# yeyupiaoling/VoiceprintRecognition-Pytorch

Measured on NVIDIA H100. Metric: embeddings/sec (3s@16kHz) ECAPA-TDNN, higher is better.
Workload: dtype f32

## Files before the change

voiceprintrecognition-pytorch_b200/csrc/api.cu:

```cuda
#include <cmath>
#include <cstdarg>
#include <cstdio>
#include <cstdlib>
#include <cstring>
#include <new>
#include <string>
#include <vector>

#include "kernels.cuh"


using namespace vpb;

struct vp_handle {
  int device = 0;
  std::string err;
  float* d_weights = nullptr;
  size_t weights_bytes = 0;
  char* d_arena = nullptr;
  size_t arena_bytes = 0;
  cudaStream_t cap_stream = nullptr;
  bool fe_set = false;
  vp_frontend_desc fe{};
  vp_frontend_options fe_opt{VP_FRAME_DEFAULT, 0, 1.0};
  float* d_window = nullptr;
  double2* d_twiddle = nullptr;
  int* d_mel_start = nullptr;
  int* d_mel_count = nullptr;
  int* d_mel_off = nullptr;
  float* d_mel_w = nullptr;
  float* d_dct = nullptr;
};

struct vp_program {
  vp_handle* h = nullptr;
  std::vector<vp_op> ops;
  std::vector<int> engines;
  size_t ws_bytes = 0, in_floats = 0, out_floats = 0;
  int launches = 0;
  int B = 0;
  cudaGraphExec_t gexec = nullptr;
  const float* g_feats = nullptr;
  float* g_emb = nullptr;
  char* g_arena = nullptr;
  int runs = 0, g_miss = 0;
  bool g_off = false;
  int n_slots = 0;
  size_t arena_need() const { return ws_bytes + (((size_t)n_slots * 4 + 255) & ~(size_t)255); }
  unsigned* slot(int32_t q) const { return q > 0 ? reinterpret_cast<unsigned*>(h->d_arena + ws_bytes) + (q - 1) : nullptr; }
};

static int fail(vp_handle* h, int code, const char* fmt, ...) {
  char buf[512];
// ... 80 lines not shown
  if (d->power != 1 && d->power != 2) return fail(h, VP_ERR_UNSUPPORTED, "power must be 1 or 2");
  if (d->use_log < 0 || d->use_log > 3) return fail(h, VP_ERR_INVALID, "use_log %d", d->use_log);
  if (d->post != 0 && d->post != 1) return fail(h, VP_ERR_INVALID, "post %d", d->post);
  if (d->post == 1) {
    if (d->kind != 1) return fail(h, VP_ERR_UNSUPPORTED, "MFCC needs stft framing");
    if (!dct) return fail(h, VP_ERR_INVALID, "MFCC needs the DCT matrix");
    if (d->n_mels > 128 || d->n_out < 1 || d->n_out > d->n_mels)
      return fail(h, VP_ERR_UNSUPPORTED, "MFCC: n_mels %d (<= 128), n_out %d (<= n_mels)", d->n_mels, d->n_out);
  }
  for (int m = 0; m < d->n_mels; ++m) {
    if (mel_count[m] < 0 || mel_start[m] < 0 || mel_start[m] + mel_count[m] > N / 2 + 1 || mel_off[m] < 0 ||
        mel_off[m] + mel_count[m] > n_w)
      return fail(h, VP_ERR_INVALID, "mel filter %d out of range", m);
  }
  CUDA_TRY(h, cudaSetDevice(h->device));
  free_frontend(h);
  std::vector<double2> tw(N);
  for (int k = 0; k < N; ++k) {
    double a = -2.0 * M_PI * (double)k / (double)N;
    tw[k] = make_double2(cos(a), sin(a));
  }
  const int F = d->n_mels;
  CUDA_TRY(h, cudaMalloc(&h->d_window, sizeof(float) * d->win_length));
  CUDA_TRY(h, cudaMalloc(&h->d_twiddle, sizeof(double2) * N));
  CUDA_TRY(h, cudaMalloc(&h->d_mel_start, sizeof(int) * F));
  CUDA_TRY(h, cudaMalloc(&h->d_mel_count, sizeof(int) * F));
  CUDA_TRY(h, cudaMalloc(&h->d_mel_off, sizeof(int) * F));
  CUDA_TRY(h, cudaMalloc(&h->d_mel_w, sizeof(float) * (n_w > 0 ? n_w : 1)));
  CUDA_TRY(h, cudaMemcpy(h->d_window, window, sizeof(float) * d->win_length, cudaMemcpyHostToDevice));
  CUDA_TRY(h, cudaMemcpy(h->d_twiddle, tw.data(), sizeof(double2) * N, cudaMemcpyHostToDevice));
  CUDA_TRY(h, cudaMemcpy(h->d_mel_start, mel_start, sizeof(int) * F, cudaMemcpyHostToDevice));
  CUDA_TRY(h, cudaMemcpy(h->d_mel_count, mel_count, sizeof(int) * F, cudaMemcpyHostToDevice));
  CUDA_TRY(h, cudaMemcpy(h->d_mel_off, mel_off, sizeof(int) * F, cudaMemcpyHostToDevice));
  if (n_w > 0) CUDA_TRY(h, cudaMemcpy(h->d_mel_w, mel_w, sizeof(float) * n_w, cudaMemcpyHostToDevice));
  if (d->post == 1) {
    CUDA_TRY(h, cudaMalloc(&h->d_dct, sizeof(float) * F * d->n_out));
    CUDA_TRY(h, cudaMemcpy(h->d_dct, dct, sizeof(float) * F * d->n_out, cudaMemcpyHostToDevice));
  }
  h->fe = *d;
  h->fe_opt = vp_frontend_options{VP_FRAME_DEFAULT, 0, 1.0};
  h->fe_set = true;
  return VP_OK;
}

int vp_frontend_set_options(vp_handle* h, const vp_frontend_options* o) {
  if (!h || !o) return fail(h, VP_ERR_INVALID, "null argument");
  if (!h->fe_set) return fail(h, VP_ERR_INVALID, "front-end not configured (vp_frontend_set)");
  const bool kaldi = h->fe.kind == 0;
  const int m = o->frame_mode;
  if (kaldi ? (m != VP_FRAME_DEFAULT && m != VP_FRAME_KALDI_REFLECT)
            : (m != VP_FRAME_DEFAULT && (m < VP_FRAME_STFT_CONSTANT || m > VP_FRAME_STFT_NOCENTER)))
    return fail(h, VP_ERR_INVALID, "frame mode %d does not fit front-end kind %d", m, h->fe.kind);
  if (o->pad < 0 || (kaldi && o->pad != 0)) return fail(h, VP_ERR_INVALID, "pad %d (kind 1 only, >= 0)", o->pad);
  if (!(o->spec_scale > 0.0) || !std::isfinite(o->spec_scale) || (kaldi && o->spec_scale != 1.0))
    return fail(h, VP_ERR_INVALID, "spec_scale %g (finite, > 0; 1 for kind 0)", o->spec_scale);
  h->fe_opt = *o;
  return VP_OK;
// ... 35 lines not shown
  size_t nblk = (T + FPB - 1) / FPB;
  size_t n = round4((size_t)B * nblk * vp_feature_dim(h));
  if (h->fe.post == 1) n += round4((size_t)B * nblk) + round4((size_t)B * T * h->fe.n_mels);
  return n;
}

static int run_frontend(vp_handle* h, int want_kind, int want_post, const float* wave, int B, int L, const int32_t* keep,
                        float* feats, float* scratch, cudaStream_t st, int stage = 0, float* ext_max = nullptr) {
  if (!h) return VP_ERR_INVALID;
  if (!h->fe_set) return fail(h, VP_ERR_INVALID, "front-end not configured (vp_frontend_set)");
  if (want_kind >= 0 && h->fe.kind != want_kind) return fail(h, VP_ERR_INVALID, "front-end kind mismatch");
  if (want_post >= 0 && h->fe.post != want_post) return fail(h, VP_ERR_INVALID, "front-end post-stage mismatch (vp_melspec vs vp_mfcc)");
  if ((stage != 2 && !wave) || (stage != 1 && !feats) || !scratch || B < 1) return fail(h, VP_ERR_INVALID, "null/empty argument");
  if (stage != 0 && (h->fe.post != 1 || !ext_max)) return fail(h, VP_ERR_INVALID, "two-stage calls are for the MFCC front-end");
  const char* len_err = frontend_length_error(h, L);
  if (*len_err) return fail(h, VP_ERR_INVALID, "waveform of %d samples: %s", L, len_err);
  const int T = vp_num_frames(h, L);
  if (T < 1) return fail(h, VP_ERR_INVALID, "waveform of %d samples is shorter than one frame (%d)", L, h->fe.win_length);
  CUDA_TRY(h, cudaSetDevice(h->device));
  FrontendParams p;
  p.wave = wave; p.feats = feats; p.partial = scratch;
  p.window = h->d_window; p.twiddle = h->d_twiddle;
  p.mel_start = h->d_mel_start; p.mel_count = h->d_mel_count; p.mel_off = h->d_mel_off; p.mel_w = h->d_mel_w;
  p.B = B; p.L = L; p.T = T; p.kind = h->fe.kind; p.N = h->fe.n_fft; p.WL = h->fe.win_length; p.hop = h->fe.hop;
  p.F = h->fe.n_mels; p.remove_dc = h->fe.remove_dc; p.power = h->fe.power; p.use_log = h->fe.use_log;
  p.fpb = FPB; p.nblk = (T + FPB - 1) / FPB;
  p.frame = h->fe_opt.frame_mode;
  p.pad = p.kind == 0 ? p.WL / 2 - p.hop / 2 : h->fe_opt.pad;
  p.spec_mult = h->fe.power == 2 ? h->fe_opt.spec_scale * h->fe_opt.spec_scale : h->fe_opt.spec_scale;
  p.preemph = h->fe.preemph; p.log_floor = h->fe.log_floor; p.db_mult = h->fe.db_mult; p.cta_max = nullptr;
  frontend_plan(p);
  if (h->fe.post == 1) {
    MfccParams m;
    float* cta_max = scratch + round4((size_t)B * p.nblk * h->fe.n_out);
    float* mel = cta_max + round4((size_t)B * p.nblk);
    p.feats = mel; p.partial = nullptr; p.cta_max = cta_max;
    m.mel = mel; m.cta_max = cta_max; m.dct = h->d_dct; m.feats = feats; m.partial = scratch;
    m.B = B; m.T = T; m.M = h->fe.n_mels; m.K = h->fe.n_out; m.fpb = FPB; m.nblk = p.nblk; m.n_max = B * p.nblk;
    m.top_db = h->fe.top_db;
    if (stage == 1) {
      CUDA_TRY(h, launch_frontend_mfcc_mel(p, ext_max, st));
    } else if (stage == 2) {
      m.cta_max = ext_max; m.n_max = 1;
      CUDA_TRY(h, launch_frontend_mfcc_finish(p, m, keep, st));
    } else {
      CUDA_TRY(h, launch_frontend_mfcc(p, m, keep, st));
    }
    return VP_OK;
  }
  CUDA_TRY(h, launch_frontend(p, keep, st));
  return VP_OK;
}

int vp_fbank(vp_handle* h, const float* wave, int32_t B, int32_t Lpad, const int32_t* keep, float* feats,
             float* scratch, void* stream) {
  return run_frontend(h, 0, 0, wave, B, Lpad, keep, feats, scratch, (cudaStream_t)stream);
}
int vp_melspec(vp_handle* h, const float* wave, int32_t B, int32_t Lpad, const int32_t* keep, float* feats,
               float* scratch, void* stream) {
  return run_frontend(h, 1, 0, wave, B, Lpad, keep, feats, scratch, (cudaStream_t)stream);
}
int vp_mfcc(vp_handle* h, const float* wave, int32_t B, int32_t Lpad, const int32_t* keep, float* feats,
            float* scratch, void* stream) {
  return run_frontend(h, 1, 1, wave, B, Lpad, keep, feats, scratch, (cudaStream_t)stream);
}

int vp_mfcc_mel(vp_handle* h, const float* wave, int32_t B, int32_t Lpad, float* scratch, float* max_out, void* stream) {
  return run_frontend(h, 1, 1, wave, B, Lpad, nullptr, nullptr, scratch, (cudaStream_t)stream, 1, max_out);
}
int vp_mfcc_finish(vp_handle* h, int32_t B, int32_t Lpad, const int32_t* keep, float* feats, float* scratch,
                   const float* max_in, void* stream) {
  return run_frontend(h, 1, 1, nullptr, B, Lpad, keep, feats, scratch, (cudaStream_t)stream, 2, const_cast<float*>(max_in));
// ... 579 lines not shown
```

voiceprintrecognition-pytorch_b200/csrc/frontend.cu:

```cuda
#include "kernels.cuh"

namespace vpb {

struct cd { double x, y; };
__device__ __forceinline__ cd cadd(cd a, cd b) { return {a.x + b.x, a.y + b.y}; }
__device__ __forceinline__ cd csub(cd a, cd b) { return {a.x - b.x, a.y - b.y}; }
__device__ __forceinline__ cd cmul(cd a, cd b) { return {a.x * b.x - a.y * b.y, a.x * b.y + a.y * b.x}; }
__device__ __forceinline__ cd cmi(cd a) { return {a.y, -a.x}; }
__device__ __forceinline__ cd ld2(const double2* p) { const double2 v = *p; return {v.x, v.y}; }
__device__ __forceinline__ void st2(double2* p, cd v) { *p = make_double2(v.x, v.y); }

__device__ __forceinline__ void group_sync(int g, int G) { asm volatile("bar.sync %0, %1;" ::"r"(g + 1), "r"(G) : "memory"); }

__global__ void __launch_bounds__(256) frontend_kernel(const __grid_constant__ FrontendParams p) {
  pdl_launch_dependents();
  pdl_wait();
  extern __shared__ __align__(16) unsigned char smem_raw[];
  const int N = p.N, WL = p.WL, F = p.F;
  const int G = p.G;
  const int NG = 256 / G;
  const int span = (p.fpb - 1) * p.hop + WL;

  double2* tw = reinterpret_cast<double2*>(smem_raw);
  double2* bufA = tw + N;
  double2* bufB = bufA + (size_t)NG * N;
  float* stage = reinterpret_cast<float*>(bufB + (size_t)NG * N);
  float* win = stage + ((span + 3) & ~3);
  float* means = win + ((WL + 3) & ~3);
  float* red = means + NG * 2;

  const int tid = threadIdx.x;
  const int b = blockIdx.y;
  const int f0 = blockIdx.x * p.fpb;
  const int g = tid / G;
  const int t = tid - g * G;
  float vmax = -INFINITY;
  const float* wv = p.wave + (size_t)b * p.L;

  const int q0 = f0 * p.hop;
  for (int i = tid; i < span; i += 256) {
    int s = q0 + i;
    if (p.kind == 1) {
      const int Lp = p.L + 2 * p.pad;
      if (p.frame != VP_FRAME_STFT_NOCENTER) s -= N / 2;
      if (p.frame == VP_FRAME_DEFAULT) {
        if (s < 0) s = -s;
        if (s >= Lp) s = 2 * (Lp - 1) - s;
      } else if (p.frame == VP_FRAME_STFT_REPLICATE) {
        s = min(max(s, 0), Lp - 1);
      } else if (p.frame == VP_FRAME_STFT_CIRCULAR) {
        if (s < 0) s += Lp;
        if (s >= Lp) s -= Lp;
      }
      s -= p.pad;
    } else if (p.frame == VP_FRAME_KALDI_REFLECT) {
      s -= p.pad;
      if (s < 0) s = -1 - s;
      if (s >= p.L) s = 2 * p.L - 1 - s;
    }
    stage[i] = (s >= 0 && s < p.L) ? __ldg(wv + s) : 0.f;
  }
  for (int i = tid; i < WL; i += 256) win[i] = __ldg(p.window + i);
  for (int i = tid; i < N; i += 256) tw[i] = __ldg(p.twiddle + i);
  __syncthreads();

  const int npairs = p.fpb / 2;
  double2* src0 = bufA + (size_t)g * N;
  double2* dst0 = bufB + (size_t)g * N;
  for (int pair = g; pair < npairs; pair += NG) {
    const int fa = f0 + pair * 2;
    const int oa = (fa - f0) * p.hop;
    const bool va = fa < p.T, vb = fa + 1 < p.T;
    if (!va) break;

    float ma = 0.f, mb = 0.f;
    if (p.kind == 0 && p.remove_dc) {
      const int w = t >> 5, lane = t & 31;
      if (G >= 64) {
        if (w < 2) {
          const int o = oa + w * p.hop;
          float s = 0.f;
          if (w == 0 || vb)
            for (int j = lane; j < WL; j += 32) s += stage[o + j];
          s = warp_sum(s);
          if (lane == 0) means[g * 2 + w] = s / (float)WL;
        }
      } else {
        for (int w2 = 0; w2 < 2; ++w2) {
          const int o = oa + w2 * p.hop;
          float s = 0.f;
          if (w2 == 0 || vb)
            for (int j = lane; j < WL; j += 32) s += stage[o + j];
          s = warp_sum(s);
          if (lane == 0) means[g * 2 + w2] = s / (float)WL;
        }
      }
      group_sync(g, G);
      ma = means[g * 2];
      mb = means[g * 2 + 1];
    }
    for (int j = t; j < N; j += G) {
      float ya = 0.f, yb = 0.f;
      if (j < WL) {
        const int jp = j > 0 ? j - 1 : 0;
        const float wj = win[j];
        {
          float x = stage[oa + j];
          if (p.kind == 0) {
            x = __fsub_rn(x, ma);
            if (p.preemph != 0.f) x = __fsub_rn(x, __fmul_rn(p.preemph, __fsub_rn(stage[oa + jp], ma)));
          }
          ya = __fmul_rn(x, wj);
        }
        if (vb) {
          float x = stage[oa + p.hop + j];
          if (p.kind == 0) {
            x = __fsub_rn(x, mb);
            if (p.preemph != 0.f) x = __fsub_rn(x, __fmul_rn(p.preemph, __fsub_rn(stage[oa + p.hop + jp], mb)));
          }
          yb = __fmul_rn(x, wj);
        }
      }
      src0[j] = make_double2((double)ya, (double)yb);
    }
    group_sync(g, G);

    double2* src = src0;
    double2* dst = dst0;
    int Ns = 1;
    for (int ps = 0; ps < p.n_pass; ++ps) {
      const int R = p.radix[ps];
      const int q = N / R;
      const int step = q / Ns;
      const bool pow2 = (Ns & (Ns - 1)) == 0;
      for (int j = t; j < q; j += G) {
        const int kk = pow2 ? (j & (Ns - 1)) : (j % Ns);
        const int base = (j - kk) * R + kk;
        if (R == 8) {
          cd v[8];
#pragma unroll
          for (int r = 0; r < 8; ++r) {
            v[r] = ld2(src + j + r * q);
            if (r > 0 && Ns > 1) v[r] = cmul(v[r], ld2(tw + r * kk * step));
          }
          const cd a0 = cadd(v[0], v[4]), a1 = csub(v[0], v[4]), a2 = cadd(v[2], v[6]), a3 = cmi(csub(v[2], v[6]));
          const cd a4 = cadd(v[1], v[5]), a5 = csub(v[1], v[5]), a6 = cadd(v[3], v[7]), a7 = cmi(csub(v[3], v[7]));
          const cd b0 = cadd(a0, a2), b2 = csub(a0, a2), b1 = cadd(a1, a3), b3 = csub(a1, a3);
          const cd b4 = cadd(a4, a6), b6 = cmi(csub(a4, a6));
          const double h = 0.70710678118654752440;
          const cd s5 = cadd(a5, a7), d5 = csub(a5, a7);
          const cd b5 = {h * (s5.x + s5.y), h * (s5.y - s5.x)};
          const cd b7 = {h * (d5.y - d5.x), -h * (d5.x + d5.y)};
          st2(dst + base, cadd(b0, b4));          st2(dst + base + Ns, cadd(b1, b5));
          st2(dst + base + 2 * Ns, cadd(b2, b6)); st2(dst + base + 3 * Ns, cadd(b3, b7));
          st2(dst + base + 4 * Ns, csub(b0, b4)); st2(dst + base + 5 * Ns, csub(b1, b5));
          st2(dst + base + 6 * Ns, csub(b2, b6)); st2(dst + base + 7 * Ns, csub(b3, b7));
        } else if (R == 4) {
          cd v0 = ld2(src + j), v1 = ld2(src + j + q), v2 = ld2(src + j + 2 * q), v3 = ld2(src + j + 3 * q);
          if (Ns > 1) {
            v1 = cmul(v1, ld2(tw + kk * step));
            v2 = cmul(v2, ld2(tw + 2 * kk * step));
            v3 = cmul(v3, ld2(tw + 3 * kk * step));
          }
          const cd a0 = cadd(v0, v2), a1 = csub(v0, v2), a2 = cadd(v1, v3), a3 = cmi(csub(v1, v3));
          st2(dst + base, cadd(a0, a2));          st2(dst + base + Ns, cadd(a1, a3));
          st2(dst + base + 2 * Ns, csub(a0, a2)); st2(dst + base + 3 * Ns, csub(a1, a3));
        } else if (R == 2) {
          const cd v0 = ld2(src + j);
          cd v1 = ld2(src + j + q);
          if (Ns > 1) v1 = cmul(v1, ld2(tw + kk * step));
          st2(dst + base, cadd(v0, v1));
          st2(dst + base + Ns, csub(v0, v1));
        } else {
          cd v[5];
#pragma unroll
          for (int r = 0; r < 5; ++r)
            if (r < R) {
              v[r] = ld2(src + j + r * q);
              if (r > 0 && Ns > 1) v[r] = cmul(v[r], ld2(tw + r * kk * step));
            }
#pragma unroll
          for (int m = 0; m < 5; ++m)
            if (m < R) {
              cd acc = v[0];
#pragma unroll
              for (int r = 1; r < 5; ++r)
                if (r < R) acc = cadd(acc, cmul(v[r], ld2(tw + ((r * m) % R) * q)));
              st2(dst + base + m * Ns, acc);
            }
        }
      }
      group_sync(g, G);
      double2* tmp = src; src = dst; dst = tmp;
      Ns *= R;
    }

    const int NB = N / 2 + 1;
    double* P = reinterpret_cast<double*>(dst);
    for (int k = t; k < NB; k += G) {
      const cd z = ld2(src + k);
      const cd zn = ld2(src + (k == 0 ? 0 : N - k));
      const double ar = 0.5 * (z.x + zn.x), ai = 0.5 * (z.y - zn.y);
      const double br = 0.5 * (z.y + zn.y), bi = -0.5 * (z.x - zn.x);
      double pa = ar * ar + ai * ai, pb = br * br + bi * bi;
      if (p.power == 1) { pa = sqrt(pa); pb = sqrt(pb); }
      if (p.spec_mult != 1.0) { pa *= p.spec_mult; pb *= p.spec_mult; }
      P[k] = pa;
      P[NB + k] = pb;
    }
    group_sync(g, G);

#pragma unroll
    for (int fr = 0; fr < 2; ++fr) {
      if (fr == 1 && !vb) break;
      const int f = fa + fr;
      const double* pf = P + fr * NB;
      for (int m = t; m < F; m += G) {
        const int st = __ldg(p.mel_start + m), cnt = __ldg(p.mel_count + m), off = __ldg(p.mel_off + m);
        double acc = 0.0;
        for (int i = 0; i < cnt; ++i) acc = fma(pf[st + i], (double)__ldg(p.mel_w + off + i), acc);
        float s = (float)acc;
        if (p.use_log == 1) s = logf(fmaxf(s, p.log_floor));
        else if (p.use_log == 2) s = p.db_mult * log10f(fmaxf(s, p.log_floor));
        else if (p.use_log == 3) s = logf(s + p.log_floor);
        vmax = fmaxf(vmax, s);
        p.feats[((size_t)b * p.T + f) * F + m] = s;
      }
    }
    group_sync(g, G);
  }
  __syncthreads();

  if (p.cta_max) {
    vmax = warp_max(vmax);
    if ((tid & 31) == 0) red[tid >> 5] = vmax;
    __syncthreads();
    if (tid == 0) {
      float m = red[0];
      for (int i = 1; i < 8; ++i) m = fmaxf(m, red[i]);
      p.cta_max[(size_t)b * p.nblk + blockIdx.x] = m;
    }
    return;
  }
  for (int m = tid; m < F; m += 256) {
    float s = 0.f;
    for (int f = f0; f < f0 + p.fpb && f < p.T; ++f) s += p.feats[((size_t)b * p.T + f) * F + m];
    p.partial[((size_t)b * p.nblk + blockIdx.x) * F + m] = s;
  }
}

__global__ void __launch_bounds__(256) mfcc_post_kernel(const __grid_constant__ MfccParams p) {
  pdl_launch_dependents();
  pdl_wait();
  extern __shared__ __align__(16) float sm[];
  float* dct = sm;
  float* tile = dct + p.M * p.K;
  float* outt = tile + p.fpb * p.M;
  float* red = outt + p.fpb * p.K;
  const int tid = threadIdx.x;
  const int b = blockIdx.y;
  const int f0 = blockIdx.x * p.fpb;
  float thr = -INFINITY;
  if (p.top_db >= 0.f) {
    float m = -INFINITY;
    for (int i = tid; i < p.n_max; i += 256) m = fmaxf(m, __ldg(p.cta_max + i));
    m = warp_max(m);
    if ((tid & 31) == 0) red[tid >> 5] = m;
    __syncthreads();
    m = red[0];
    for (int i = 1; i < 8; ++i) m = fmaxf(m, red[i]);
// ... 14 lines not shown
    for (int m = 0; m < p.M; ++m) s = fmaf(row[m], dct[m * p.K + k], s);
    outt[i] = s;
    if (f0 + fr < p.T) p.feats[((size_t)b * p.T + f0 + fr) * p.K + k] = s;
  }
  __syncthreads();
  for (int k = tid; k < p.K; k += 256) {
    float s = 0.f;
    for (int fr = 0; fr < p.fpb && f0 + fr < p.T; ++fr) s += outt[fr * p.K + k];
    p.partial[((size_t)b * p.nblk + blockIdx.x) * p.K + k] = s;
  }
}

__global__ void __launch_bounds__(128) cmn_mask_kernel(float* feats, const float* partial, const int* keep, int T, int F,
                                                       int nblk, int rows_per_cta) {
  pdl_launch_dependents();
  pdl_wait();
  const int b = blockIdx.y;
  const int kp = keep ? keep[b] : T;
  const int t0 = blockIdx.x * rows_per_cta;
  for (int m = threadIdx.x; m < F; m += blockDim.x) {
    float s = 0.f;
    for (int i = 0; i < nblk; ++i) s += partial[((size_t)b * nblk + i) * F + m];
    const float mean = s / (float)T;
    for (int t = t0; t < t0 + rows_per_cta && t < T; ++t) {
      float* q = feats + ((size_t)b * T + t) * F + m;
      *q = (t < kp) ? (*q - mean) : 0.f;
    }
  }
}

__global__ void __launch_bounds__(256) max_reduce_kernel(const float* v, int n, float* out) {
  pdl_launch_dependents();
  pdl_wait();
  __shared__ float red[8];
  float m = -INFINITY;
  for (int i = threadIdx.x; i < n; i += 256) m = fmaxf(m, v[i]);
  m = warp_max(m);
  if ((threadIdx.x & 31) == 0) red[threadIdx.x >> 5] = m;
  __syncthreads();
  if (threadIdx.x == 0) {
    m = red[0];
    for (int i = 1; i < 8; ++i) m = fmaxf(m, red[i]);
    out[0] = m;
  }
}

static int frontend_group_threads(int N) {
  const int first = (N % 8 == 0) ? 8 : 4;
  int G = ((N / first + 31) / 32) * 32;
  if (G < 32) G = 32;
  if (G > 256) G = 256;
  while (256 % G) G += 32;
  return G;
}

void frontend_plan(FrontendParams& p) {
  int n = p.N, k = 0;
  for (int r : {8, 4, 2, 5, 3})
    while (n % r == 0 && k < 12) { p.radix[k++] = r; n /= r; }
  p.n_pass = k;
  p.G = frontend_group_threads(p.N);
}

size_t frontend_smem_bytes(int N, int WL, int hop, int fpb) {
  const int G = frontend_group_threads(N);
  const int NG = 256 / G;
  const int span = (fpb - 1) * hop + WL;
  return sizeof(double2) * ((size_t)N + 2 * (size_t)NG * N) + sizeof(float) * (((span + 3) & ~3) + ((WL + 3) & ~3) + 2 * NG + 8 + 4);
}

static cudaError_t ensure_frontend_smem(size_t smem) {
  static PerDeviceSmem once;
  if (once.need(smem)) {
    cudaError_t e = cudaFuncSetAttribute(frontend_kernel, cudaFuncAttributeMaxDynamicSharedMemorySize, (int)smem);
    if (e != cudaSuccess) return e;
    once.set(smem);
  }
  return cudaSuccess;
}

cudaError_t launch_frontend_mfcc_mel(const FrontendParams& p, float* max_out, cudaStream_t stream) {
  size_t smem = frontend_smem_bytes(p.N, p.WL, p.hop, p.fpb);
  cudaError_t e = ensure_frontend_smem(smem);
  if (e != cudaSuccess) return e;
  dim3 grid(p.nblk, p.B);
  launch_pdl(frontend_kernel, grid, 256, smem, stream, p);
  e = cudaGetLastError();
  if (e != cudaSuccess) return e;
  launch_pdl(max_reduce_kernel, 1, 256, 0, stream, p.cta_max, p.B * p.nblk, max_out);
  return cudaGetLastError();
}

cudaError_t launch_frontend_mfcc_finish(const FrontendParams& p, const MfccParams& m, const int* keep, cudaStream_t stream) {
  dim3 grid(p.nblk, p.B);
  size_t smem2 = ((size_t)m.M * m.K + (size_t)m.fpb * (m.M + m.K) + 8) * sizeof(float);
  static PerDeviceSmem once;
  cudaError_t e;
  if (once.need(smem2)) {
    e = cudaFuncSetAttribute(mfcc_post_kernel, cudaFuncAttributeMaxDynamicSharedMemorySize, (int)smem2);
    if (e != cudaSuccess) return e;
    once.set(smem2);
  }
  launch_pdl(mfcc_post_kernel, grid, 256, smem2, stream, m);
  e = cudaGetLastError();
  if (e != cudaSuccess) return e;
  const int rows = 64;
  dim3 g2((p.T + rows - 1) / rows, p.B);
  launch_pdl(cmn_mask_kernel, g2, 128, 0, stream, m.feats, m.partial, keep, p.T, m.K, p.nblk, rows);
  return cudaGetLastError();
}

cudaError_t launch_frontend_mfcc(const FrontendParams& p, const MfccParams& m, const int* keep, cudaStream_t stream) {
  size_t smem = frontend_smem_bytes(p.N, p.WL, p.hop, p.fpb);
  cudaError_t e = ensure_frontend_smem(smem);
  if (e != cudaSuccess) return e;
  dim3 grid(p.nblk, p.B);
  launch_pdl(frontend_kernel, grid, 256, smem, stream, p);
  e = cudaGetLastError();
  if (e != cudaSuccess) return e;
  return launch_frontend_mfcc_finish(p, m, keep, stream);
}

cudaError_t launch_frontend(const FrontendParams& p, const int* keep, cudaStream_t stream) {
  size_t smem = frontend_smem_bytes(p.N, p.WL, p.hop, p.fpb);
  cudaError_t e = ensure_frontend_smem(smem);
  if (e != cudaSuccess) return e;
  dim3 grid(p.nblk, p.B);
  launch_pdl(frontend_kernel, grid, 256, smem, stream, p);
  e = cudaGetLastError();
  if (e != cudaSuccess) return e;
  const int rows = 64;
  dim3 g2((p.T + rows - 1) / rows, p.B);
  launch_pdl(cmn_mask_kernel, g2, 128, 0, stream, p.feats, p.partial, keep, p.T, p.F, p.nblk, rows);
  return cudaGetLastError();
}

}
```

voiceprintrecognition-pytorch_b200/csrc/kernels.cuh:

```cuda
#pragma once
#include "common.cuh"

namespace vpb {

struct FrontendParams {
  const float* wave; float* feats; float* partial;
  const float* window; const double2* twiddle;
  const int* mel_start; const int* mel_count; const int* mel_off; const float* mel_w;
  int B, L, T, kind, N, WL, hop, F, remove_dc, power, use_log, fpb, nblk;
  int frame;
  int pad;
  double spec_mult;
  float preemph, log_floor, db_mult;
  float* cta_max;
  int n_pass, radix[12], G;
};
void frontend_plan(FrontendParams& p);

struct MfccParams {
  const float* mel; const float* cta_max; const float* dct; float* feats; float* partial;
  int B, T, M, K, fpb, nblk, n_max;
  float top_db;
};

struct StatsParams {
  const float* src; float* dst;
  int B, R, C, in_ld, in_coff, out_ld, out_coff, mode, seg_len, n_seg;
  float eps;
};

struct AspParams {
  const float* x; const float* logit; float* dst;
  int B, T, C, x_ld, x_coff, l_ld, l_coff, out_ld, out_coff, mean_only;
  float eps;
};

struct EwParams {
  const float* x; const float* y; const float* att; const float* gate; const float* res; float* dst;
  long long rows; int C, rows_per_utt;
  int x_ld, x_coff, y_ld, y_coff, att_ld, att_coff, res_ld, res_coff, out_ld, out_coff, mode, act2;
// ... 14 lines not shown
int spectral_launches_tridiag(int n);
int apply_q_max_rows(int kz);
cudaError_t launch_spectral_laplacian(const float* emb, int n, int D, int n_drop, double* L, void* scratch, cudaStream_t stream);
cudaError_t launch_sym_tridiag(double* A, int n, double* d, double* e, double* tau, void* scratch, cudaStream_t stream);
cudaError_t launch_sym_tridiag_apply_q(const double* A, const double* tau, int n, double* Z, int kz, cudaStream_t stream);

size_t verify_scratch_bytes(int64_t n);
cudaError_t launch_verify_sort(const float* scores, const int32_t* labels, const int32_t* trial, const int32_t* enroll,
                               int64_t n_enroll, int64_t n, void* scratch, cudaStream_t stream);
cudaError_t launch_verify_curve(int64_t n, double p_target, double c_miss, double c_fa, void* scratch, float* sorted_scores,
                                uint8_t* sorted_labels, vp_verify_result* result, cudaStream_t stream);

cudaError_t launch_resample(const float* x, int64_t in_ld, float* y, int64_t out_ld, int B, const int64_t* n_in,
                            const int64_t* n_out, const int32_t* up, const int32_t* down, const int64_t* tap_off,
                            const double* taps, cudaStream_t stream);
size_t gain_scratch_bytes(int B, int64_t ld);
cudaError_t launch_gain(float* w, int64_t ld, int B, const int64_t* lens, double target_db, double max_gain_db,
                        int32_t* flags, void* scratch, cudaStream_t stream);

cudaError_t launch_frontend(const FrontendParams& p, const int* keep, cudaStream_t stream);
cudaError_t launch_frontend_mfcc(const FrontendParams& p, const MfccParams& m, const int* keep, cudaStream_t stream);
cudaError_t launch_frontend_mfcc_mel(const FrontendParams& p, float* max_out, cudaStream_t stream);
cudaError_t launch_frontend_mfcc_finish(const FrontendParams& p, const MfccParams& m, const int* keep, cudaStream_t stream);
size_t frontend_smem_bytes(int N, int WL, int hop, int fpb);
cudaError_t launch_conv_ffma(const ConvParams& p, cudaStream_t stream);
cudaError_t launch_conv_c1(const ConvParams& p, cudaStream_t stream);
cudaError_t launch_colstats(const StatsParams& p, cudaStream_t stream);
cudaError_t launch_asp_pool(const AspParams& p, cudaStream_t stream);
cudaError_t launch_ew(const EwParams& p, cudaStream_t stream);
bool conv_tc_supported(const ConvParams& p);
cudaError_t launch_conv_tc(const ConvParams& p, cudaStream_t stream);
bool conv_tc16_supported(const ConvParams& p);
cudaError_t launch_conv_tc16(const ConvParams& p, const float* w_tc16, float descale, cudaStream_t stream);

}
```

Measured before the change: 29300.

## Rewrite frontend FFT kernel with templated register FFT, padded smem and multi-tile CTAs

Reworks the fbank/mel frontend kernel: adds compile-time-N specializations that keep the FFT in registers with padded shared buffers and per-stage precomputed twiddles, caches mel weights and indices in shared memory, and loads constants via cp.async before the PDL wait. It also lets one CTA process several frame tiles, caching features in smem for the mean partials, and batches the mean-subtraction loop. The goal is to cut bank conflicts, global loads and launch/tail overhead in the feature extraction stage. It adds more shared memory per CTA, which may reduce occupancy.

```diff
diff --git a/voiceprintrecognition-pytorch_b200/csrc/api.cu b/voiceprintrecognition-pytorch_b200/csrc/api.cu
--- a/voiceprintrecognition-pytorch_b200/csrc/api.cu
+++ b/voiceprintrecognition-pytorch_b200/csrc/api.cu
@@ -28,7 +28,8 @@
   int* d_mel_start = nullptr;
   int* d_mel_count = nullptr;
   int* d_mel_off = nullptr;
-  float* d_mel_w = nullptr;
+  double* d_mel_w = nullptr;
+  int mel_nw = 0;
   float* d_dct = nullptr;
 };
 
@@ -155,17 +156,21 @@
   }
   const int F = d->n_mels;
   CUDA_TRY(h, cudaMalloc(&h->d_window, sizeof(float) * d->win_length));
-  CUDA_TRY(h, cudaMalloc(&h->d_twiddle, sizeof(double2) * N));
+  std::vector<double2> twx(N + 8);
+  frontend_twiddle_table(N, tw.data(), twx.data());
+  std::vector<double> mel_wd(mel_w, mel_w + (n_w > 0 ? n_w : 0));
+  CUDA_TRY(h, cudaMalloc(&h->d_twiddle, sizeof(double2) * (N + 8)));
   CUDA_TRY(h, cudaMalloc(&h->d_mel_start, sizeof(int) * F));
   CUDA_TRY(h, cudaMalloc(&h->d_mel_count, sizeof(int) * F));
   CUDA_TRY(h, cudaMalloc(&h->d_mel_off, sizeof(int) * F));
-  CUDA_TRY(h, cudaMalloc(&h->d_mel_w, sizeof(float) * (n_w > 0 ? n_w : 1)));
+  CUDA_TRY(h, cudaMalloc(&h->d_mel_w, sizeof(double) * (n_w > 0 ? n_w : 1)));
   CUDA_TRY(h, cudaMemcpy(h->d_window, window, sizeof(float) * d->win_length, cudaMemcpyHostToDevice));
-  CUDA_TRY(h, cudaMemcpy(h->d_twiddle, tw.data(), sizeof(double2) * N, cudaMemcpyHostToDevice));
+  CUDA_TRY(h, cudaMemcpy(h->d_twiddle, twx.data(), sizeof(double2) * (N + 8), cudaMemcpyHostToDevice));
   CUDA_TRY(h, cudaMemcpy(h->d_mel_start, mel_start, sizeof(int) * F, cudaMemcpyHostToDevice));
   CUDA_TRY(h, cudaMemcpy(h->d_mel_count, mel_count, sizeof(int) * F, cudaMemcpyHostToDevice));
   CUDA_TRY(h, cudaMemcpy(h->d_mel_off, mel_off, sizeof(int) * F, cudaMemcpyHostToDevice));
-  if (n_w > 0) CUDA_TRY(h, cudaMemcpy(h->d_mel_w, mel_w, sizeof(float) * n_w, cudaMemcpyHostToDevice));
+  if (n_w > 0) CUDA_TRY(h, cudaMemcpy(h->d_mel_w, mel_wd.data(), sizeof(double) * n_w, cudaMemcpyHostToDevice));
+  h->mel_nw = n_w > 0 ? n_w : 0;
   if (d->post == 1) {
     CUDA_TRY(h, cudaMalloc(&h->d_dct, sizeof(float) * F * d->n_out));
     CUDA_TRY(h, cudaMemcpy(h->d_dct, dct, sizeof(float) * F * d->n_out, cudaMemcpyHostToDevice));
@@ -247,6 +252,7 @@
   p.wave = wave; p.feats = feats; p.partial = scratch;
   p.window = h->d_window; p.twiddle = h->d_twiddle;
   p.mel_start = h->d_mel_start; p.mel_count = h->d_mel_count; p.mel_off = h->d_mel_off; p.mel_w = h->d_mel_w;
+  p.mel_nw = h->mel_nw;
   p.B = B; p.L = L; p.T = T; p.kind = h->fe.kind; p.N = h->fe.n_fft; p.WL = h->fe.win_length; p.hop = h->fe.hop;
   p.F = h->fe.n_mels; p.remove_dc = h->fe.remove_dc; p.power = h->fe.power; p.use_log = h->fe.use_log;
   p.fpb = FPB; p.nblk = (T + FPB - 1) / FPB;
@@ -254,12 +260,12 @@
   p.pad = p.kind == 0 ? p.WL / 2 - p.hop / 2 : h->fe_opt.pad;
   p.spec_mult = h->fe.power == 2 ? h->fe_opt.spec_scale * h->fe_opt.spec_scale : h->fe_opt.spec_scale;
   p.preemph = h->fe.preemph; p.log_floor = h->fe.log_floor; p.db_mult = h->fe.db_mult; p.cta_max = nullptr;
-  frontend_plan(p);
   if (h->fe.post == 1) {
     MfccParams m;
     float* cta_max = scratch + round4((size_t)B * p.nblk * h->fe.n_out);
     float* mel = cta_max + round4((size_t)B * p.nblk);
     p.feats = mel; p.partial = nullptr; p.cta_max = cta_max;
+    frontend_plan(p);
     m.mel = mel; m.cta_max = cta_max; m.dct = h->d_dct; m.feats = feats; m.partial = scratch;
     m.B = B; m.T = T; m.M = h->fe.n_mels; m.K = h->fe.n_out; m.fpb = FPB; m.nblk = p.nblk; m.n_max = B * p.nblk;
     m.top_db = h->fe.top_db;
@@ -273,6 +279,7 @@
     }
     return VP_OK;
   }
+  frontend_plan(p);
   CUDA_TRY(h, launch_frontend(p, keep, st));
   return VP_OK;
 }
diff --git a/voiceprintrecognition-pytorch_b200/csrc/frontend.cu b/voiceprintrecognition-pytorch_b200/csrc/frontend.cu
--- a/voiceprintrecognition-pytorch_b200/csrc/frontend.cu
+++ b/voiceprintrecognition-pytorch_b200/csrc/frontend.cu
@@ -10,35 +10,139 @@
 __device__ __forceinline__ cd ld2(const double2* p) { const double2 v = *p; return {v.x, v.y}; }
 __device__ __forceinline__ void st2(double2* p, cd v) { *p = make_double2(v.x, v.y); }
 
+__device__ __forceinline__ int xpad(int i) { return i + (i >> 3); }
+static int xpad_len(int N) { return N + (N >> 3); }
+
+template <int BYTES>
+__device__ __forceinline__ void cp_async(void* dst, const void* src) {
+  const unsigned d = (unsigned)__cvta_generic_to_shared(dst);
+  if (BYTES == 16) asm volatile("cp.async.cg.shared.global [%0], [%1], 16;" ::"r"(d), "l"(src) : "memory");
+  else asm volatile("cp.async.ca.shared.global [%0], [%1], %2;" ::"r"(d), "l"(src), "n"(BYTES) : "memory");
+}
+__device__ __forceinline__ void cp_async_wait_all() { asm volatile("cp.async.wait_all;" ::: "memory"); }
+
 __device__ __forceinline__ void group_sync(int g, int G) { asm volatile("bar.sync %0, %1;" ::"r"(g + 1), "r"(G) : "memory"); }
 
-__global__ void __launch_bounds__(256) frontend_kernel(const __grid_constant__ FrontendParams p) {
+__device__ __forceinline__ void bfly8(const cd* v, cd* o) {
+  const cd a0 = cadd(v[0], v[4]), a1 = csub(v[0], v[4]), a2 = cadd(v[2], v[6]), a3 = cmi(csub(v[2], v[6]));
+  const cd a4 = cadd(v[1], v[5]), a5 = csub(v[1], v[5]), a6 = cadd(v[3], v[7]), a7 = cmi(csub(v[3], v[7]));
+  const cd b0 = cadd(a0, a2), b2 = csub(a0, a2), b1 = cadd(a1, a3), b3 = csub(a1, a3);
+  const cd b4 = cadd(a4, a6), b6 = cmi(csub(a4, a6));
+  const double h = 0.70710678118654752440;
+  const cd s5 = cadd(a5, a7), d5 = csub(a5, a7);
+  const cd b5 = {h * (s5.x + s5.y), h * (s5.y - s5.x)};
+  const cd b7 = {h * (d5.y - d5.x), -h * (d5.x + d5.y)};
+  o[0] = cadd(b0, b4); o[1] = cadd(b1, b5); o[2] = cadd(b2, b6); o[3] = cadd(b3, b7);
+  o[4] = csub(b0, b4); o[5] = csub(b1, b5); o[6] = csub(b2, b6); o[7] = csub(b3, b7);
+}
+__device__ __forceinline__ void bfly4(const cd* v, cd* o) {
+  const cd a0 = cadd(v[0], v[2]), a1 = csub(v[0], v[2]), a2 = cadd(v[1], v[3]), a3 = cmi(csub(v[1], v[3]));
+  o[0] = cadd(a0, a2); o[1] = cadd(a1, a3); o[2] = csub(a0, a2); o[3] = csub(a1, a3);
+}
+__device__ __forceinline__ void bfly2(const cd* v, cd* o) {
+  o[0] = cadd(v[0], v[1]);
+  o[1] = csub(v[0], v[1]);
+}
+template <int R>
+__device__ __forceinline__ void bfly(const cd* v, cd* o) {
+  if (R == 8) bfly8(v, o);
+  else if (R == 4) bfly4(v, o);
+  else bfly2(v, o);
+}
+
+__host__ __device__ constexpr int pow2_radix(int rem) { return rem % 8 == 0 ? 8 : (rem % 4 == 0 ? 4 : 2); }
+__host__ __device__ constexpr int pow2_last_radix(int N) { return pow2_radix(N) == N ? N : pow2_last_radix(N / pow2_radix(N)); }
+__host__ __device__ constexpr int pow2_passes(int N) { return N == 1 ? 0 : 1 + pow2_passes(N / pow2_radix(N)); }
+
+template <int N, int Ns>
+__device__ __forceinline__ double2* fft_pow2(cd (&v)[8], double2* src, double2* dst, const double2* twx, int t, int g) {
+  constexpr int G = N / 8, R = pow2_radix(N / Ns), q = N / R, nb = 8 / R;
+  constexpr bool last = Ns * R == N;
+  if (Ns > 1) {
+#pragma unroll
+    for (int i = 0; i < nb; ++i)
+#pragma unroll
+      for (int r = 0; r < R; ++r) v[i * R + r] = ld2(src + xpad(t + i * G + r * q));
+  }
+#pragma unroll
+  for (int i = 0; i < nb; ++i) {
+    const int j = t + i * G;
+    const int kk = j & (Ns - 1);
+    if (Ns > 1) {
+#pragma unroll
+      for (int r = 1; r < R; ++r) v[i * R + r] = cmul(v[i * R + r], ld2(twx + (Ns - 1) + (r - 1) * Ns + kk));
+    }
+    cd o[R];
+    bfly<R>(&v[i * R], o);
+    const int base = (j - kk) * R + kk;
+#pragma unroll
+    for (int m = 0; m < R; ++m) {
+      v[i * R + m] = o[m];
+      if (!last) st2(dst + xpad(base + m * Ns), o[m]);
+      else if (i * G + m * Ns >= N / 2) st2(dst + j + m * Ns, o[m]);
+    }
+  }
+  group_sync(g, G);
+  if constexpr (last) return dst;
+  else return fft_pow2<N, Ns * R>(v, dst, src, twx, t, g);
+}
+
+__device__ __forceinline__ void split_power(const FrontendParams& p, cd z, cd zn, double& pa, double& pb) {
+  const double ar = 0.5 * (z.x + zn.x), ai = 0.5 * (z.y - zn.y);
+  const double br = 0.5 * (z.y + zn.y), bi = -0.5 * (z.x - zn.x);
+  pa = ar * ar + ai * ai;
+  pb = br * br + bi * bi;
+  if (p.power == 1) { pa = sqrt(pa); pb = sqrt(pb); }
+  if (p.spec_mult != 1.0) { pa *= p.spec_mult; pb *= p.spec_mult; }
+}
+
+template <int NFFT>
+__global__ void __launch_bounds__(256, 2) frontend_kernel(const __grid_constant__ FrontendParams p) {
   pdl_launch_dependents();
-  pdl_wait();
   extern __shared__ __align__(16) unsigned char smem_raw[];
-  const int N = p.N, WL = p.WL, F = p.F;
-  const int G = p.G;
+  const int N = NFFT ? NFFT : p.N, WL = p.WL, F = p.F;
+  const int G = NFFT ? NFFT / 8 : p.G;
   const int NG = 256 / G;
-  const int span = (p.fpb - 1) * p.hop + WL;
-
-  double2* tw = reinterpret_cast<double2*>(smem_raw);
-  double2* bufA = tw + N;
-  double2* bufB = bufA + (size_t)NG * N;
-  float* stage = reinterpret_cast<float*>(bufB + (size_t)NG * N);
+  const int cfr = p.fpb * p.tpc;
+  const int span = (cfr - 1) * p.hop + WL;
+  const int XN = N + (N >> 3);
+
+  double2* twx = reinterpret_cast<double2*>(smem_raw);
+  double2* roots = twx + N;
+  double2* bufs = roots + 8;
+  double* melw = reinterpret_cast<double*>(bufs + (size_t)NG * 2 * XN);
+  float* stage = reinterpret_cast<float*>(melw + ((p.mel_nw + 1) & ~1));
   float* win = stage + ((span + 3) & ~3);
-  float* means = win + ((WL + 3) & ~3);
+  float* fcache = win + ((WL + 3) & ~3);
+  int* melidx = reinterpret_cast<int*>(fcache + (p.cache ? (size_t)cfr * F : 0));
+  float* means = reinterpret_cast<float*>(melidx + 3 * F);
   float* red = means + NG * 2;
 
   const int tid = threadIdx.x;
   const int b = blockIdx.y;
-  const int f0 = blockIdx.x * p.fpb;
+  const int f0 = blockIdx.x * cfr;
   const int g = tid / G;
   const int t = tid - g * G;
   float vmax = -INFINITY;
   const float* wv = p.wave + (size_t)b * p.L;
 
+  for (int i = tid; i < N + 8; i += 256) cp_async<16>(twx + i, p.twiddle + i);
+  for (int i = tid; i < p.mel_nw; i += 256) cp_async<8>(melw + i, p.mel_w + i);
+  for (int i = tid; i < WL; i += 256) cp_async<4>(win + i, p.window + i);
+  for (int i = tid; i < F; i += 256) {
+    cp_async<4>(melidx + i, p.mel_start + i);
+    cp_async<4>(melidx + F + i, p.mel_count + i);
+    cp_async<4>(melidx + 2 * F + i, p.mel_off + i);
+  }
+  pdl_wait();
   const int q0 = f0 * p.hop;
-  for (int i = tid; i < span; i += 256) {
+  int i0 = 0;
+  if (p.kind == 0 && p.frame != VP_FRAME_KALDI_REFLECT && (reinterpret_cast<size_t>(wv + q0) & 15) == 0) {
+    const int n4 = min(span, p.L - q0) >> 2;
+    for (int i = tid; i < n4; i += 256) cp_async<16>(stage + 4 * i, wv + q0 + 4 * i);
+    i0 = n4 * 4;
+  }
+  for (int i = i0 + tid; i < span; i += 256) {
     int s = q0 + i;
     if (p.kind == 1) {
       const int Lp = p.L + 2 * p.pad;
@@ -60,13 +164,13 @@
     }
     stage[i] = (s >= 0 && s < p.L) ? __ldg(wv + s) : 0.f;
   }
-  for (int i = tid; i < WL; i += 256) win[i] = __ldg(p.window + i);
-  for (int i = tid; i < N; i += 256) tw[i] = __ldg(p.twiddle + i);
+  cp_async_wait_all();
   __syncthreads();
 
-  const int npairs = p.fpb / 2;
-  double2* src0 = bufA + (size_t)g * N;
-  double2* dst0 = bufB + (size_t)g * N;
+  const int npairs = cfr / 2;
+  double2* bufA = bufs + (size_t)g * 2 * XN;
+  double2* bufB = bufA + XN;
+  const int NB = N / 2 + 1;
   for (int pair = g; pair < npairs; pair += NG) {
     const int fa = f0 + pair * 2;
     const int oa = (fa - f0) * p.hop;
@@ -99,7 +203,7 @@
       ma = means[g * 2];
       mb = means[g * 2 + 1];
     }
-    for (int j = t; j < N; j += G) {
+    auto windowed = [&](int j) -> cd {
       float ya = 0.f, yb = 0.f;
       if (j < WL) {
         const int jp = j > 0 ? j - 1 : 0;
@@ -121,131 +225,168 @@
           yb = __fmul_rn(x, wj);
         }
       }
-      src0[j] = make_double2((double)ya, (double)yb);
+      return {(double)ya, (double)yb};
+    };
+
+    double* P;
+    if constexpr (NFFT != 0) {
+      cd v[8];
+#pragma unroll
+      for (int r = 0; r < 8; ++r) v[r] = windowed(t + r * (NFFT / 8));
+      const double2* zbuf = fft_pow2<NFFT, 1>(v, bufB, bufA, twx, t, g);
+      P = reinterpret_cast<double*>(zbuf == bufA ? bufB : bufA);
+      constexpr int LR = pow2_last_radix(NFFT), LNs = NFFT / LR;
+#pragma unroll
+      for (int i = 0; i < 8 / LR; ++i)
+#pragma unroll
+        for (int m = 0; m < LR; ++m) {
+          constexpr int Gc = NFFT / 8;
+          const int kb = i * Gc + m * LNs;
+          if (kb < NFFT / 2 || (kb == NFFT / 2 && t == 0)) {
+            const int k = t + kb;
+            const cd z = v[i * LR + m];
+            const cd zn = (k == 0 || kb == NFFT / 2) ? z : ld2(zbuf + (NFFT - k));
+            double pa, pb;
+            split_power(p, z, zn, pa, pb);
+            P[k] = pa;
+            P[NB + k] = pb;
+          }
+        }
+    } else {
+      for (int j = t; j < N; j += G) st2(bufA + xpad(j), windowed(j));
+      group_sync(g, G);
+      double2* src = bufA;
+      double2* dst = bufB;
+      int Ns = 1;
+      for (int ps = 0; ps < p.n_pass; ++ps) {
+        const int R = p.radix[ps];
+        const int q = N / R;
+        const bool pow2 = (Ns & (Ns - 1)) == 0;
+        for (int j = t; j < q; j += G) {
+          const int kk = pow2 ? (j & (Ns - 1)) : (j % Ns);
+          const int base = (j - kk) * R + kk;
+          const double2* tq = twx + (Ns - 1) + kk - Ns;
+          if (R == 8 || R == 4 || R == 2) {
+            cd v[8], o[8];
+#pragma unroll
+            for (int r = 0; r < 8; ++r)
+              if (r < R) {
+                v[r] = ld2(src + xpad(j + r * q));
+                if (r > 0 && Ns > 1) v[r] = cmul(v[r], ld2(tq + r * Ns));
+              }
+            if (R == 8) bfly8(v, o);
+            else if (R == 4) bfly4(v, o);
+            else bfly2(v, o);
+#pragma unroll
+            for (int m = 0; m < 8; ++m)
+              if (m < R) st2(dst + xpad(base + m * Ns), o[m]);
+          } else {
+            const double2* wr = roots + (R == 5 ? 0 : 5);
+            cd v[5];
+#pragma unroll
+            for (int r = 0; r < 5; ++r)
+              if (r < R) {
+                v[r] = ld2(src + xpad(j + r * q));
+                if (r > 0 && Ns > 1) v[r] = cmul(v[r], ld2(tq + r * Ns));
+              }
+#pragma unroll
+            for (int m = 0; m < 5; ++m)
+              if (m < R) {
+                cd acc = v[0];
+#pragma unroll
+                for (int r = 1; r < 5; ++r)
+                  if (r < R) acc = cadd(acc, cmul(v[r], ld2(wr + (r * m) % R)));
+                st2(dst + xpad(base + m * Ns), acc);
+              }
+          }
+        }
+        group_sync(g, G);
+        double2* tmp = src; src = dst; dst = tmp;
+        Ns *= R;
+      }
+      P = reinterpret_cast<double*>(dst);
+      for (int k = t; k < NB; k += G) {
+        double pa, pb;
+        split_power(p, ld2(src + xpad(k)), ld2(src + xpad(k == 0 ? 0 : N - k)), pa, pb);
+        P[k] = pa;
+        P[NB + k] = pb;
+      }
     }
     group_sync(g, G);
 
-    double2* src = src0;
-    double2* dst = dst0;
-    int Ns = 1;
-    for (int ps = 0; ps < p.n_pass; ++ps) {
-      const int R = p.radix[ps];
-      const int q = N / R;
-      const int step = q / Ns;
-      const bool pow2 = (Ns & (Ns - 1)) == 0;
-      for (int j = t; j < q; j += G) {
-        const int kk = pow2 ? (j & (Ns - 1)) : (j % Ns);
-        const int base = (j - kk) * R + kk;
-        if (R == 8) {
-          cd v[8];
-#pragma unroll
-          for (int r = 0; r < 8; ++r) {
-            v[r] = ld2(src + j + r * q);
-            if (r > 0 && Ns > 1) v[r] = cmul(v[r], ld2(tw + r * kk * step));
-          }
-          const cd a0 = cadd(v[0], v[4]), a1 = csub(v[0], v[4]), a2 = cadd(v[2], v[6]), a3 = cmi(csub(v[2], v[6]));
-          const cd a4 = cadd(v[1], v[5]), a5 = csub(v[1], v[5]), a6 = cadd(v[3], v[7]), a7 = cmi(csub(v[3], v[7]));
-          const cd b0 = cadd(a0, a2), b2 = csub(a0, a2), b1 = cadd(a1, a3), b3 = csub(a1, a3);
-          const cd b4 = cadd(a4, a6), b6 = cmi(csub(a4, a6));
-          const double h = 0.70710678118654752440;
-          const cd s5 = cadd(a5, a7), d5 = csub(a5, a7);
-          const cd b5 = {h * (s5.x + s5.y), h * (s5.y - s5.x)};
-          const cd b7 = {h * (d5.y - d5.x), -h * (d5.x + d5.y)};
-          st2(dst + base, cadd(b0, b4));          st2(dst + base + Ns, cadd(b1, b5));
-          st2(dst + base + 2 * Ns, cadd(b2, b6)); st2(dst + base + 3 * Ns, cadd(b3, b7));
-          st2(dst + base + 4 * Ns, csub(b0, b4)); st2(dst + base + 5 * Ns, csub(b1, b5));
-          st2(dst + base + 6 * Ns, csub(b2, b6)); st2(dst + base + 7 * Ns, csub(b3, b7));
-        } else if (R == 4) {
-          cd v0 = ld2(src + j), v1 = ld2(src + j + q), v2 = ld2(src + j + 2 * q), v3 = ld2(src + j + 3 * q);
-          if (Ns > 1) {
-            v1 = cmul(v1, ld2(tw + kk * step));
-            v2 = cmul(v2, ld2(tw + 2 * kk * step));
-            v3 = cmul(v3, ld2(tw + 3 * kk * step));
-          }
-          const cd a0 = cadd(v0, v2), a1 = csub(v0, v2), a2 = cadd(v1, v3), a3 = cmi(csub(v1, v3));
-          st2(dst + base, cadd(a0, a2));          st2(dst + base + Ns, cadd(a1, a3));
-          st2(dst + base + 2 * Ns, csub(a0, a2)); st2(dst + base + 3 * Ns, csub(a1, a3));
-        } else if (R == 2) {
-          const cd v0 = ld2(src + j);
-          cd v1 = ld2(src + j + q);
-          if (Ns > 1) v1 = cmul(v1, ld2(tw + kk * step));
-          st2(dst + base, cadd(v0, v1));
-          st2(dst + base + Ns, csub(v0, v1));
-        } else {
-          cd v[5];
-#pragma unroll
-          for (int r = 0; r < 5; ++r)
-            if (r < R) {
-              v[r] = ld2(src + j + r * q);
-              if (r > 0 && Ns > 1) v[r] = cmul(v[r], ld2(tw + r * kk * step));
-            }
-#pragma unroll
-          for (int m = 0; m < 5; ++m)
-            if (m < R) {
-              cd acc = v[0];
-#pragma unroll
-              for (int r = 1; r < 5; ++r)
-                if (r < R) acc = cadd(acc, cmul(v[r], ld2(tw + ((r * m) % R) * q)));
-              st2(dst + base + m * Ns, acc);
-            }
-        }
-      }
-      group_sync(g, G);
-      double2* tmp = src; src = dst; dst = tmp;
-      Ns *= R;
-    }
-
-    const int NB = N / 2 + 1;
-    double* P = reinterpret_cast<double*>(dst);
-    for (int k = t; k < NB; k += G) {
-      const cd z = ld2(src + k);
-      const cd zn = ld2(src + (k == 0 ? 0 : N - k));
-      const double ar = 0.5 * (z.x + zn.x), ai = 0.5 * (z.y - zn.y);
-      const double br = 0.5 * (z.y + zn.y), bi = -0.5 * (z.x - zn.x);
-      double pa = ar * ar + ai * ai, pb = br * br + bi * bi;
-      if (p.power == 1) { pa = sqrt(pa); pb = sqrt(pb); }
-      if (p.spec_mult != 1.0) { pa *= p.spec_mult; pb *= p.spec_mult; }
-      P[k] = pa;
-      P[NB + k] = pb;
-    }
-    group_sync(g, G);
-
-#pragma unroll
-    for (int fr = 0; fr < 2; ++fr) {
-      if (fr == 1 && !vb) break;
-      const int f = fa + fr;
-      const double* pf = P + fr * NB;
-      for (int m = t; m < F; m += G) {
-        const int st = __ldg(p.mel_start + m), cnt = __ldg(p.mel_count + m), off = __ldg(p.mel_off + m);
+    auto emit = [&](int o, double acc) {
+      const int fr = o >= F, m = o - fr * F;
+      float s = (float)acc;
+      if (p.use_log == 1) s = logf(fmaxf(s, p.log_floor));
+      else if (p.use_log == 2) s = p.db_mult * log10f(fmaxf(s, p.log_floor));
+      else if (p.use_log == 3) s = logf(s + p.log_floor);
+      vmax = fmaxf(vmax, s);
+      p.feats[((size_t)b * p.T + fa + fr) * F + m] = s;
+      if (p.cache) fcache[(size_t)(fa + fr - f0) * F + m] = s;
+    };
+    constexpr int MU = 4;
+    if (NFFT == 0 || 2 * F <= G) {
+      for (int o = t; o < 2 * F && (o < F || vb); o += G) {
+        const int fr = o >= F, m = o - fr * F;
+        const double* pf = P + fr * NB + melidx[m];
+        const double* wf = melw + melidx[2 * F + m];
+        const int cnt = melidx[F + m];
         double acc = 0.0;
-        for (int i = 0; i < cnt; ++i) acc = fma(pf[st + i], (double)__ldg(p.mel_w + off + i), acc);
-        float s = (float)acc;
-        if (p.use_log == 1) s = logf(fmaxf(s, p.log_floor));
-        else if (p.use_log == 2) s = p.db_mult * log10f(fmaxf(s, p.log_floor));
-        else if (p.use_log == 3) s = logf(s + p.log_floor);
-        vmax = fmaxf(vmax, s);
-        p.feats[((size_t)b * p.T + f) * F + m] = s;
-      }
-    }
-    group_sync(g, G);
+        for (int i = 0; i < cnt; ++i) acc = fma(pf[i], wf[i], acc);
+        emit(o, acc);
+      }
+    } else {
+      for (int o0 = t; o0 < 2 * F; o0 += MU * G) {
+        const double* pf[MU];
+        const double* wf[MU];
+        int cnt[MU], cmax = 0;
+        double acc[MU];
+#pragma unroll
+        for (int u = 0; u < MU; ++u) {
+          const int o = o0 + u * G, fr = o >= F;
+          const bool live = o < 2 * F && (!fr || vb);
+          const int m = live ? o - fr * F : 0;
+          pf[u] = P + fr * NB + melidx[m];
+          wf[u] = melw + melidx[2 * F + m];
+          cnt[u] = live ? melidx[F + m] : 0;
+          cmax = max(cmax, cnt[u]);
+          acc[u] = 0.0;
+        }
+        for (int i = 0; i < cmax; ++i)
+#pragma unroll
+          for (int u = 0; u < MU; ++u)
+            if (i < cnt[u]) acc[u] = fma(pf[u][i], wf[u][i], acc[u]);
+#pragma unroll
+        for (int u = 0; u < MU; ++u) {
+          const int o = o0 + u * G;
+          if (o < 2 * F && (o < F || vb)) emit(o, acc[u]);
+        }
+      }
+    }
+    if (NFFT == 0 || pow2_passes(NFFT ? NFFT : 1) % 2 == 0) group_sync(g, G);
   }
   __syncthreads();
 
+  const int blk0 = blockIdx.x * p.tpc;
   if (p.cta_max) {
     vmax = warp_max(vmax);
     if ((tid & 31) == 0) red[tid >> 5] = vmax;
     __syncthreads();
-    if (tid == 0) {
+    if (tid < p.tpc && blk0 + tid < p.nblk) {
       float m = red[0];
       for (int i = 1; i < 8; ++i) m = fmaxf(m, red[i]);
-      p.cta_max[(size_t)b * p.nblk + blockIdx.x] = m;
+      p.cta_max[(size_t)b * p.nblk + blk0 + tid] = m;
     }
     return;
   }
-  for (int m = tid; m < F; m += 256) {
+  for (int i = tid; i < p.tpc * F; i += 256) {
+    const int ti = i / F, m = i - ti * F;
+    if (blk0 + ti >= p.nblk) break;
+    const int fb = f0 + ti * p.fpb;
     float s = 0.f;
-    for (int f = f0; f < f0 + p.fpb && f < p.T; ++f) s += p.feats[((size_t)b * p.T + f) * F + m];
-    p.partial[((size_t)b * p.nblk + blockIdx.x) * F + m] = s;
+    for (int f = fb; f < fb + p.fpb && f < p.T; ++f)
+      s += p.cache ? fcache[(size_t)(f - f0) * F + m] : p.feats[((size_t)b * p.T + f) * F + m];
+    p.partial[((size_t)b * p.nblk + blk0 + ti) * F + m] = s;
   }
 }
 
@@ -306,9 +447,15 @@
     float s = 0.f;
     for (int i = 0; i < nblk; ++i) s += partial[((size_t)b * nblk + i) * F + m];
     const float mean = s / (float)T;
-    for (int t = t0; t < t0 + rows_per_cta && t < T; ++t) {
-      float* q = feats + ((size_t)b * T + t) * F + m;
-      *q = (t < kp) ? (*q - mean) : 0.f;
+    const int t1 = min(t0 + rows_per_cta, T);
+    for (int tb = t0; tb < t1; tb += 16) {
+      float v[16];
+#pragma unroll
+      for (int u = 0; u < 16; ++u)
+        if (tb + u < t1 && tb + u < kp) v[u] = feats[((size_t)b * T + tb + u) * F + m];
+#pragma unroll
+      for (int u = 0; u < 16; ++u)
+        if (tb + u < t1) feats[((size_t)b * T + tb + u) * F + m] = (tb + u < kp) ? (v[u] - mean) : 0.f;
     }
   }
 }
@@ -338,38 +485,72 @@
   return G;
 }
 
+static int plan_radices(int N, int* radix) {
+  int n = N, k = 0;
+  for (int r : {8, 4, 2, 5, 3})
+    while (n % r == 0 && k < 12) { radix[k++] = r; n /= r; }
+  return k;
+}
+
+void frontend_twiddle_table(int N, const double2* tw, double2* out) {
+  int radix[12];
+  const int n_pass = plan_radices(N, radix);
+  int Ns = 1;
+  for (int ps = 0; ps < n_pass; Ns *= radix[ps++])
+    for (int r = 1; r < radix[ps]; ++r)
+      for (int kk = 0; kk < Ns; ++kk) out[(Ns - 1) + (r - 1) * Ns + kk] = tw[r * kk * (N / (Ns * radix[ps]))];
+  out[N - 1] = make_double2(0.0, 0.0);
+  for (int k = 0; k < 8; ++k) {
+    const int R = k < 5 ? 5 : 3, e = k < 5 ? k : k - 5;
+    out[N + k] = (N % R == 0) ? tw[e * (N / R)] : make_double2(0.0, 0.0);
+  }
+}
+
+static size_t frontend_smem_bytes(const FrontendParams& p, int tpc, bool cache) {
+  const int NG = 256 / p.G;
+  const int cfr = p.fpb * tpc;
+  const int span = (cfr - 1) * p.hop + p.WL;
+  return sizeof(double2) * ((size_t)p.N + 8 + 2 * (size_t)NG * xpad_len(p.N)) + sizeof(double) * ((p.mel_nw + 1) & ~1) +
+         sizeof(float) * (((span + 3) & ~3) + ((p.WL + 3) & ~3) + (cache ? (size_t)cfr * p.F : 0) + 3 * p.F + 2 * NG + 8);
+}
+
 void frontend_plan(FrontendParams& p) {
-  int n = p.N, k = 0;
-  for (int r : {8, 4, 2, 5, 3})
-    while (n % r == 0 && k < 12) { p.radix[k++] = r; n /= r; }
-  p.n_pass = k;
+  p.n_pass = plan_radices(p.N, p.radix);
   p.G = frontend_group_threads(p.N);
-}
-
-size_t frontend_smem_bytes(int N, int WL, int hop, int fpb) {
-  const int G = frontend_group_threads(N);
-  const int NG = 256 / G;
-  const int span = (fpb - 1) * hop + WL;
-  return sizeof(double2) * ((size_t)N + 2 * (size_t)NG * N) + sizeof(float) * (((span + 3) & ~3) + ((WL + 3) & ~3) + 2 * NG + 8 + 4);
-}
-
-static cudaError_t ensure_frontend_smem(size_t smem) {
+  const size_t half_sm = (228 * 1024 - 2 * 1024) / 2, cta_max = 227 * 1024;
+  const bool want = p.cta_max == nullptr;
+  p.tpc = 1;
+  p.cache = want && frontend_smem_bytes(p, 1, true) <= cta_max;
+  for (int tpc : {4, 2})
+    if (tpc <= p.nblk && frontend_smem_bytes(p, tpc, want) <= half_sm) { p.tpc = tpc; p.cache = want; break; }
+}
+
+template <int NFFT>
+static cudaError_t launch_frontend_kernel_n(const FrontendParams& p, size_t smem, cudaStream_t stream) {
   static PerDeviceSmem once;
   if (once.need(smem)) {
-    cudaError_t e = cudaFuncSetAttribute(frontend_kernel, cudaFuncAttributeMaxDynamicSharedMemorySize, (int)smem);
+    cudaError_t e = cudaFuncSetAttribute(frontend_kernel<NFFT>, cudaFuncAttributeMaxDynamicSharedMemorySize, (int)smem);
     if (e != cudaSuccess) return e;
     once.set(smem);
   }
-  return cudaSuccess;
+  dim3 grid((p.nblk + p.tpc - 1) / p.tpc, p.B);
+  launch_pdl(frontend_kernel<NFFT>, grid, 256, smem, stream, p);
+  return cudaGetLastError();
+}
+
+static cudaError_t launch_frontend_kernel(const FrontendParams& p, cudaStream_t stream) {
+  const size_t smem = frontend_smem_bytes(p, p.tpc, p.cache);
+  switch (p.N) {
+    case 256: return launch_frontend_kernel_n<256>(p, smem, stream);
+    case 512: return launch_frontend_kernel_n<512>(p, smem, stream);
+    case 1024: return launch_frontend_kernel_n<1024>(p, smem, stream);
+    case 2048: return launch_frontend_kernel_n<2048>(p, smem, stream);
+    default: return launch_frontend_kernel_n<0>(p, smem, stream);
+  }
 }
 
 cudaError_t launch_frontend_mfcc_mel(const FrontendParams& p, float* max_out, cudaStream_t stream) {
-  size_t smem = frontend_smem_bytes(p.N, p.WL, p.hop, p.fpb);
-  cudaError_t e = ensure_frontend_smem(smem);
-  if (e != cudaSuccess) return e;
-  dim3 grid(p.nblk, p.B);
-  launch_pdl(frontend_kernel, grid, 256, smem, stream, p);
-  e = cudaGetLastError();
+  cudaError_t e = launch_frontend_kernel(p, stream);
   if (e != cudaSuccess) return e;
   launch_pdl(max_reduce_kernel, 1, 256, 0, stream, p.cta_max, p.B * p.nblk, max_out);
   return cudaGetLastError();
@@ -395,23 +576,13 @@
 }
 
 cudaError_t launch_frontend_mfcc(const FrontendParams& p, const MfccParams& m, const int* keep, cudaStream_t stream) {
-  size_t smem = frontend_smem_bytes(p.N, p.WL, p.hop, p.fpb);
-  cudaError_t e = ensure_frontend_smem(smem);
-  if (e != cudaSuccess) return e;
-  dim3 grid(p.nblk, p.B);
-  launch_pdl(frontend_kernel, grid, 256, smem, stream, p);
-  e = cudaGetLastError();
+  cudaError_t e = launch_frontend_kernel(p, stream);
   if (e != cudaSuccess) return e;
   return launch_frontend_mfcc_finish(p, m, keep, stream);
 }
 
 cudaError_t launch_frontend(const FrontendParams& p, const int* keep, cudaStream_t stream) {
-  size_t smem = frontend_smem_bytes(p.N, p.WL, p.hop, p.fpb);
-  cudaError_t e = ensure_frontend_smem(smem);
-  if (e != cudaSuccess) return e;
-  dim3 grid(p.nblk, p.B);
-  launch_pdl(frontend_kernel, grid, 256, smem, stream, p);
-  e = cudaGetLastError();
+  cudaError_t e = launch_frontend_kernel(p, stream);
   if (e != cudaSuccess) return e;
   const int rows = 64;
   dim3 g2((p.T + rows - 1) / rows, p.B);
diff --git a/voiceprintrecognition-pytorch_b200/csrc/kernels.cuh b/voiceprintrecognition-pytorch_b200/csrc/kernels.cuh
--- a/voiceprintrecognition-pytorch_b200/csrc/kernels.cuh
+++ b/voiceprintrecognition-pytorch_b200/csrc/kernels.cuh
@@ -6,7 +6,8 @@
 struct FrontendParams {
   const float* wave; float* feats; float* partial;
   const float* window; const double2* twiddle;
-  const int* mel_start; const int* mel_count; const int* mel_off; const float* mel_w;
+  const int* mel_start; const int* mel_count; const int* mel_off; const double* mel_w;
+  int mel_nw;
   int B, L, T, kind, N, WL, hop, F, remove_dc, power, use_log, fpb, nblk;
   int frame;
   int pad;
@@ -14,8 +15,10 @@
   float preemph, log_floor, db_mult;
   float* cta_max;
   int n_pass, radix[12], G;
+  int tpc, cache;
 };
 void frontend_plan(FrontendParams& p);
+void frontend_twiddle_table(int N, const double2* tw, double2* out);
 
 struct MfccParams {
   const float* mel; const float* cta_max; const float* dct; float* feats; float* partial;
@@ -76,7 +79,6 @@
 cudaError_t launch_frontend_mfcc(const FrontendParams& p, const MfccParams& m, const int* keep, cudaStream_t stream);
 cudaError_t launch_frontend_mfcc_mel(const FrontendParams& p, float* max_out, cudaStream_t stream);
 cudaError_t launch_frontend_mfcc_finish(const FrontendParams& p, const MfccParams& m, const int* keep, cudaStream_t stream);
-size_t frontend_smem_bytes(int N, int WL, int hop, int fpb);
 cudaError_t launch_conv_ffma(const ConvParams& p, cudaStream_t stream);
 cudaError_t launch_conv_c1(const ConvParams& p, cudaStream_t stream);
 cudaError_t launch_colstats(const StatsParams& p, cudaStream_t stream);
```

After: 30300, median of 6. 1.03x the previous value.
